# jianfch/stable-ts

Hardware: AMD Instinct MI355X
Metric: real-time factor (audio-sec/wall-sec) large-v3 word_timestamps=True (higher is better)
Workload: dtype f16; 1 GPU; large-v3 (random-init, weight recipe BENCH_WEIGHTS = the parity-pinned recipe of tests/test_gpu_f16_depth.py), 10 min synthetic 16 kHz audio per GPU, word_timestamps=True, beam_size=5, 112 decode steps/window, window-parallel batch 20, default regrouping inside the timed pass; mode=transcribe, windows_per_gpu=20, segments=125, words=1670, parallelism=dp1 (windows sharded, no data-path collective)

## Files before the change

### include/swx.h

```cpp
#ifndef SWX_H
#define SWX_H
#include <stdint.h>
#include <stddef.h>

#ifdef __cplusplus
extern "C" {
#endif

#define SWX_F32 0
#define SWX_F16 1

#define SWX_N_SAMPLES 480000
#define SWX_N_FRAMES 3000
#define SWX_N_FFT 400
#define SWX_HOP 160

typedef struct swx_dims {
    int32_t n_mels, n_audio_ctx, n_audio_state, n_audio_head, n_audio_layer;
    int32_t n_vocab, n_text_ctx, n_text_state, n_text_head, n_text_layer;
} swx_dims;

typedef struct swx_model swx_model;

const char *swx_strerror(int code);
// ... 131 lines not shown
int swx_flac_probe(const uint8_t *h_data, size_t n_bytes, swx_flac_info *info);
int64_t swx_flac_decode(const uint8_t *h_data, size_t n_bytes, int32_t *h_out, int64_t capacity_frames, swx_flac_info *info);

size_t swx_dtw_workspace_bytes(int W, int ld_n, int ld_m);
int swx_dtw(const float *d_x, int W, int ld_n, int ld_m, const int32_t *d_N, const int32_t *d_M,
            int32_t *d_text_idx, int32_t *d_time_idx, int32_t *d_len, void *d_trace_ws, void *stream);

int swx_prof_enable(int on);
int swx_debug_flags(int flags);
int swx_prof_collect(double *out, int n_classes);
int swx_graph_stats(const swx_model *m, int64_t *out);

int swx_test_gemm(int dtype, const void *d_a, int64_t lda, const void *d_w, const float *d_bias, const void *d_res,
                  void *d_c, int64_t ldc, int M, int N, int K, int epilogue, int force_kernel, void *stream);
int swx_test_gemm_plan(int M, int N, int K, int epilogue, int force_kernel, int flags);
int swx_test_dec_gemm(const void *d_a, int64_t lda, const void *d_w, const float *d_gamma, const float *d_beta,
                      const float *d_bias, void *d_c, int64_t ldc, void *d_x, void *d_kcache, void *d_vcache,
                      const int32_t *d_pos0, int n_ctx, int d, int M, int N, int K, int epilogue, void *d_scratch,
                      size_t scratch_bytes, void *stream);
int swx_test_layernorm(int dtype, const void *d_x, const float *d_g, const float *d_b, void *d_y, int rows, int d,
                       void *stream);
int swx_test_attention(int dtype, const void *d_q, int64_t ldq, const void *d_k, const void *d_v, int64_t ldkv,
                       void *d_o, int64_t ldo, int B, int H, int nq, int nk, int force_kernel, int vt_kp, void *stream);

int swx_test_gemm_layout(int dtype, const void *d_a, int64_t lda, const void *d_w, int64_t ldw, const float *d_bias, const void *d_res,
                         const float *d_resf, int res_mod, void *d_c, int64_t ldc, void *d_c2, void *d_p, int64_t p_bs, int p_nkpad,
                         int p_vcol0, int vt_s, int vt_kp, int64_t vt_bs, int vt_zero_pad, int M, int N, int K, int epilogue,
                         int force_kernel, void *stream);
int swx_test_xkv_pack(const void *d_k, const void *d_vt, void *d_packed, int B, int H, int nk, int ldk, int vt_kp, int64_t batch_stride,
                      void *stream);
// ... 56 lines not shown
```

### stable_ts_amd/_lib.py

```python
import ctypes
import os
from ctypes import POINTER, Structure, c_char_p, c_float, c_int, c_int32, c_int64, c_size_t, c_uint64, c_void_p

_HERE = os.path.dirname(os.path.abspath(__file__))
LIB_PATH = os.path.join(_HERE, "libswx.so")

SWX_F32 = 0
SWX_F16 = 1


class SwxError(RuntimeError):
    pass


class swx_dims(Structure):
    _fields_ = [(n, c_int32) for n in ("n_mels", "n_audio_ctx", "n_audio_state", "n_audio_head", "n_audio_layer",
                                       "n_vocab", "n_text_ctx", "n_text_state", "n_text_head", "n_text_layer")]


class swx_flac_info(Structure):
    _fields_ = [("sample_rate", c_int32), ("channels", c_int32), ("bits_per_sample", c_int32), ("min_block", c_int32),
                ("max_block", c_int32), ("total_samples", c_int64), ("md5", ctypes.c_uint8 * 16)]


# ... 79 lines not shown
    "swx_spectral_gate": (c_int, [c_void_p, c_int64, c_int, c_int64, POINTER(swx_gate_cfg), c_void_p, c_int64, c_void_p, c_size_t,
                                  c_void_p]),
    "swx_test_spectral_gate_block": (c_int, [c_int]),
    "swx_flac_probe": (c_int, [c_void_p, c_size_t, POINTER(swx_flac_info)]),
    "swx_flac_decode": (c_int64, [c_void_p, c_size_t, c_void_p, c_int64, POINTER(swx_flac_info)]),
    "swx_dtw_workspace_bytes": (c_size_t, [c_int, c_int, c_int]),
    "swx_dtw": (c_int, [c_void_p, c_int, c_int, c_int, c_void_p, c_void_p, c_void_p, c_void_p, c_void_p, c_void_p,
                        c_void_p]),
    "swx_prof_enable": (c_int, [c_int]),
    "swx_debug_flags": (c_int, [c_int]),
    "swx_prof_collect": (c_int, [POINTER(ctypes.c_double), c_int]),
    "swx_graph_stats": (c_int, [c_void_p, POINTER(c_int64)]),
    "swx_test_gemm": (c_int, [c_int, c_void_p, c_int64, c_void_p, c_void_p, c_void_p, c_void_p, c_int64, c_int, c_int,
                              c_int, c_int, c_int, c_void_p]),
    "swx_test_gemm_plan": (c_int, [c_int, c_int, c_int, c_int, c_int, c_int]),
    "swx_test_dec_gemm": (c_int, [c_void_p, c_int64, c_void_p, c_void_p, c_void_p, c_void_p, c_void_p, c_int64, c_void_p,
                                  c_void_p, c_void_p, c_void_p, c_int, c_int, c_int, c_int, c_int, c_int, c_void_p, c_size_t,
                                  c_void_p]),
    "swx_test_self_attn_step": (c_int, [c_void_p, c_void_p, c_void_p, c_void_p, c_void_p, c_int, c_int, c_int, c_int, c_int, c_void_p,
                                        c_void_p]),
    "swx_test_self_attn_multi": (c_int, [c_void_p, c_void_p, c_void_p, c_int, c_int, c_int, c_int, c_int, c_int, c_void_p, c_void_p]),
    "swx_test_self_attn_general": (c_int, [c_int, c_void_p, c_int64, c_void_p, c_void_p, c_void_p, c_void_p, c_int, c_int, c_int, c_int,
                                           c_int, c_int, c_int, c_int, c_void_p, c_void_p]),
    "swx_test_kcache_index": (c_int, [c_int] * 6),
    "swx_test_kcache_relayout": (c_int, [c_void_p, c_void_p, c_int64, c_int, c_int, c_int, c_int]),
    "swx_test_dec_gemm_kl": (c_int, [c_void_p, c_int64, c_void_p, c_void_p, c_void_p, c_void_p, c_void_p, c_int64, c_void_p,
                                     c_void_p, c_void_p, c_void_p, c_int, c_int, c_int, c_int, c_int, c_int, c_int, c_int, c_void_p,
                                     c_size_t, c_void_p]),
    "swx_test_self_attn_step_kl": (c_int, [c_void_p, c_void_p, c_void_p, c_void_p, c_void_p, c_int, c_int, c_int, c_int, c_int, c_int,
                                           c_void_p, c_void_p]),
# ... 64 lines not shown
```

### stable_ts_amd/csrc/swx_attn.hip

```cpp
#include <type_traits>
#include "swx_common.h"
#include "swx_kernels.h"
#include "swx_attn.h"

namespace {

constexpr int FL_KT = 64;
constexpr int FL_LD = 72;

template <bool VT, int QB>
__global__ __launch_bounds__(256, 2) void attn_flash2_f16(AttnArgs a)
{
    __shared__ __attribute__((aligned(16))) f16 Ks[2][FL_KT][FL_LD];
    __shared__ __attribute__((aligned(16))) f16 Vt[2][DH][FL_LD];
    const int tid = threadIdx.x, lane = tid & 63, wave = tid >> 6;
    const int b = blockIdx.z, h = blockIdx.y;
    const int q0 = blockIdx.x * (QB * 64) + wave * (QB * 16);
    const int qn = lane & 15, g = lane >> 4;
    const f16 *Q = (const f16 *)a.q;
    const f16 *K = (const f16 *)a.k + (size_t)b * a.k_bs + h * DH;
    const f16 *V = (const f16 *)a.v + (size_t)b * a.v_bs + (VT ? (size_t)h * DH * a.vt_kp : (size_t)h * DH);

    f16x8 qf[QB][2];
#pragma unroll
    for (int qb = 0; qb < QB; ++qb) {
// ... 68 lines not shown
            if (kt0 + FL_KT > a.nk) {
#pragma unroll
                for (int tt = 0; tt < 4; ++tt)
#pragma unroll
                    for (int r = 0; r < 4; ++r)
                        if (kt0 + tt * 16 + g * 4 + r >= a.nk) sc[tt][r] = -__builtin_inff();
            }
            float tmax = -__builtin_inff();
#pragma unroll
            for (int tt = 0; tt < 4; ++tt)
#pragma unroll
                for (int r = 0; r < 4; ++r) tmax = fmaxf(tmax, sc[tt][r]);
            tmax = lane_xor16_max(tmax);
            tmax = lane_xor32_max(tmax);
            const float m_new = fmaxf(m_run[qb], tmax);
            const float alpha = __builtin_amdgcn_exp2f((m_run[qb] - m_new) * SC2);
            const float mc = m_new * SC2;
            float psum = 0.f;
#pragma unroll
            for (int tt = 0; tt < 4; ++tt)
#pragma unroll
                for (int r = 0; r < 4; ++r) {
                    const float p = __builtin_amdgcn_exp2f(__builtin_fmaf(sc[tt][r], SC2, -mc));
                    sc[tt][r] = p;
                    psum += p;
                }
            psum = lane_xor16_add(psum);
            psum = lane_xor32_add(psum);
            l_run[qb] = l_run[qb] * alpha + psum;
            m_run[qb] = m_new;
#pragma unroll
            for (int tt = 0; tt < 4; ++tt) { o[qb][tt][0] *= alpha; o[qb][tt][1] *= alpha; o[qb][tt][2] *= alpha; o[qb][tt][3] *= alpha; }
#pragma unroll
            for (int c = 0; c < 2; ++c)
#pragma unroll
                for (int r = 0; r < 4; ++r) { pb[qb][c][r] = (f16)sc[2 * c][r]; pb[qb][c][4 + r] = (f16)sc[2 * c + 1][r]; }
        }
#pragma unroll
        for (int c = 0; c < 2; ++c)
#pragma unroll
            for (int tt = 0; tt < 4; ++tt) {
                const f16x4 lo = *(const f16x4 *)&Vt[cur][tt * 16 + qn][32 * c + g * 4];
                const f16x4 hi = *(const f16x4 *)&Vt[cur][tt * 16 + qn][32 * c + 16 + g * 4];
                f16x8 va;
#pragma unroll
                for (int e = 0; e < 4; ++e) { va[e] = lo[e]; va[4 + e] = hi[e]; }
#pragma unroll
// ... 503 lines not shown
                        part[(2 * RW_QB + qi) * DH + d] + part[(3 * RW_QB + qi) * DH + d];
        ((T *)a.o)[((size_t)b * a.q_rows_per_batch + q0 + qi) * a.ldo + h * DH + d] = from_f32<T>(v);
    }
}

}

static bool f32_flash_ready(bool vt, bool split)
{
    constexpr int need = (int)F32_LDS_BYTES;
    const hipError_t e = vt ? (split ? swx_lds_grant<attn_flash_f32<true, true>>(need) : swx_lds_grant<attn_flash_f32<true, false>>(need))
                            : (split ? swx_lds_grant<attn_flash_f32<false, true>>(need) : swx_lds_grant<attn_flash_f32<false, false>>(need));
    return e == hipSuccess;
}

int swx_attention(int dtype, const AttnArgs &a, int force_kernel, hipStream_t s)
{
    if (a.B <= 0 || a.nq <= 0 || a.nk <= 0) return 0;
    if (a.nk > RW_MAXK) return -5;
    const bool flash = (dtype == SWX_F16) && (force_kernel == 2 || (force_kernel >= 4 && force_kernel <= 6) || (force_kernel == 0 && a.nq >= 32));
    const size_t esz = dtype == SWX_F16 ? 2 : 4;
    const SwxXattnPlan xp = swx_xattn_plan(dtype, a, force_kernel, swx_flags());
    if (xp.family < 0) return xp.family;
    if (xp.family != SWX_XA_NOT_DECODE) return swx_xattn_launch(xp, a, s);
    if (flash) {
        if (dtype != SWX_F16) return -5;
        SwxProfScope prof(PC_ATTN_FLASH, 4.0 * a.B * a.H * (double)a.nq * a.nk * 64, s);
        const bool wide_fills = (int64_t)a.B * a.H * cdiv(a.nq, 256) >= 256;
        const bool narrow_fills = a.vt_kp && force_kernel == 0 && a.nq >= 256 && (int64_t)a.B * a.H * cdiv(a.nq, 128) <= 256 &&
                                  !(swx_flags() & SWX_FLAG_FLASH_NO_QB1);
        const int qb = !a.vt_kp ? 2 : narrow_fills ? 1 : force_kernel == 4 ? 2 : force_kernel == 6 ? 3 : (force_kernel == 5 || (a.nq >= 1024 && wide_fills)) ? 4 : 2;
        dim3 g(cdiv(a.nq, 64 * qb), a.H, a.B);
        const bool gen3 = a.vt_kp && (swx_flags() & SWX_FLAG_FLASH_PIPELINED);
        if (!a.vt_kp) hipLaunchKernelGGL((attn_flash2_f16<false, 2>), g, dim3(256), 0, s, a);
        else if (gen3 && qb == 4) hipLaunchKernelGGL((attn_flash3_f16<4>), g, dim3(256), 0, s, a);
        else if (gen3 && qb == 3) hipLaunchKernelGGL((attn_flash3_f16<3>), g, dim3(256), 0, s, a);
        else if (gen3 && qb == 2) hipLaunchKernelGGL((attn_flash3_f16<2>), g, dim3(256), 0, s, a);
        else if (qb == 4) hipLaunchKernelGGL((attn_flash2_f16<true, 4>), g, dim3(256), 0, s, a);
        else if (qb == 3) hipLaunchKernelGGL((attn_flash2_f16<true, 3>), g, dim3(256), 0, s, a);
        else if (qb == 1) hipLaunchKernelGGL((attn_flash2_f16<true, 1>), g, dim3(256), 0, s, a);
        else hipLaunchKernelGGL((attn_flash2_f16<true, 2>), g, dim3(256), 0, s, a);
    } else if (dtype == SWX_F32 && (force_kernel == 0 || force_kernel == 7) && a.vt_kp % F32_KT == 0 &&
               (a.vt_kp == 0 || a.vt_kp >= cdiv(a.nk, F32_KT) * F32_KT) && f32_flash_ready(a.vt_kp != 0, a.nq <= 16 && !a.f32_no_split)) {
        const bool split = a.nq <= 16 && !a.f32_no_split;
        SwxProfScope prof(split ? PC_ATTN_ROWWISE : PC_ATTN_FLASH,
                          split ? (double)a.B * a.H * 64 * esz * (2.0 * a.nk + 2.0 * a.nq) : 4.0 * a.B * a.H * (double)a.nq * a.nk * 64, s);
        dim3 gd(split ? 1 : cdiv(a.nq, 128), a.H, a.B);
        if (a.vt_kp) {
            if (split) hipLaunchKernelGGL((attn_flash_f32<true, true>), gd, dim3(256), F32_LDS_BYTES, s, a);
            else hipLaunchKernelGGL((attn_flash_f32<true, false>), gd, dim3(256), F32_LDS_BYTES, s, a);
        } else {
            if (split) hipLaunchKernelGGL((attn_flash_f32<false, true>), gd, dim3(256), F32_LDS_BYTES, s, a);
            else hipLaunchKernelGGL((attn_flash_f32<false, false>), gd, dim3(256), F32_LDS_BYTES, s, a);
        }
    } else {
        if (force_kernel == 7) return -5;
// ... 42 lines not shown
```

### stable_ts_amd/csrc/swx_gemm.hip

```cpp
#include "swx_gemm_tile.h"

namespace {

template <int MT>
__global__ __launch_bounds__(256) void gemm_f16_skinny(GemmArgs g)
{
    constexpr int NKS_MAX = 10;
    __shared__ f32x4 red[3][MT][64];
    const int tid = threadIdx.x, lane = tid & 63, wave = tid >> 6;
    const int n0 = blockIdx.x * 16;
    const f16 *A = (const f16 *)g.A;
    const f16 *W = (const f16 *)g.W;
    const int fr = lane & 15, fk = (lane >> 4) * 8;
    const int kslice = g.K / 4;
    const int nks = kslice / 32;
    const int kb = wave * kslice;
    const int n = n0 + fr;
    const bool nok = n < g.N;
    const f16 *wp = W + (size_t)(nok ? n : 0) * g.ldw + kb + fk;
    const f16x8 zero8 = (f16x8)(f16)0;

    f16x8 wf[NKS_MAX];
#pragma unroll
    for (int ks = 0; ks < NKS_MAX; ++ks) {
// ... 47 lines not shown
        }
    }
}

template <int MT = 1>
void launch_skinny(int mt, const GemmArgs &g, hipStream_t s)
{
    if constexpr (MT < 8) {
        if (mt > MT) return launch_skinny<MT + 1>(mt, g, s);
    }
    hipLaunchKernelGGL(gemm_f16_skinny<MT>, dim3(cdiv(g.N, 16)), dim3(256), 0, s, g);
}

}

int swx_gemm_plan_f16(int M, int N, int K, int epi, int64_t ldc, int64_t ldr, bool ptr16, int force_kernel, int flags)
{
    if (K % 32 != 0) return -4;
    const bool skinny_ok = M <= 128 && K % 128 == 0 && K / 128 <= 10 && N <= 16384;
    if (force_kernel == 2) return skinny_ok ? SWX_GEMM_SKINNY : -4;
    if (skinny_ok && force_kernel != 1 && force_kernel < 7) return SWX_GEMM_SKINNY;
    const bool glds_ok = K % 64 == 0 && ptr16;
    if (force_kernel >= 7 && !glds_ok) return -4;
    if (force_kernel == 1 || !glds_ok) return SWX_GEMM_TILED_REG;
    const int64_t t128 = (int64_t)cdiv(N, BN) * cdiv(M, BM);
    const bool narrow = force_kernel == 8 || (force_kernel != 9 && N % 64 == 0 && t128 < 224);
    const bool big_ok = !(epi & ~(EPI_BIAS | EPI_GELU | EPI_RES)) && ldc % 8 == 0 && (!(epi & EPI_RES) || ldr % 8 == 0);
    if (force_kernel == 12) return big_ok && K >= 128 ? SWX_GEMM_BIG : -4;
    const int64_t t256 = (int64_t)cdiv(M, BG) * cdiv(N, BG);
    const double fill = (double)t256 / (double)(((t256 + 255) / 256) * 256);
    if (force_kernel == 0 && big_ok && t256 >= 200 && K >= 512 && (fill >= 0.9 || (fill >= 0.75 && K >= 2560)) &&
        !(flags & SWX_FLAG_NO_BIG_TILE))
        return SWX_GEMM_BIG;
    const bool ring_ok = K >= 128;
    if (force_kernel == 10 || force_kernel == 11) return !ring_ok ? -4 : force_kernel == 10 ? SWX_GEMM_RING64 : SWX_GEMM_RING128;
    if (force_kernel == 0 && ring_ok && M > 256 && (narrow || t128 <= 256) && !(flags & SWX_FLAG_NO_RING))
        return narrow ? SWX_GEMM_RING64 : SWX_GEMM_RING128;
    return narrow ? SWX_GEMM_GLDS64 : SWX_GEMM_GLDS128;
}

int swx_gemm(int dtype, const GemmArgs &g, int force_kernel, hipStream_t s)
{
    if (g.M <= 0 || g.N <= 0) return 0;
    if (dtype == SWX_F16) {
        if (g.lda % 8 != 0 || g.ldw % 8 != 0) return -4;
        const bool ptr16 = (uintptr_t)g.A % 16 == 0 && (uintptr_t)g.W % 16 == 0;
        const bool cr16 = (uintptr_t)g.C % 16 == 0 && (!(g.epi & EPI_RES) || (uintptr_t)g.R % 16 == 0);
        const int plan = swx_gemm_plan_f16(g.M, g.N, g.K, g.epi, cr16 ? g.ldc : 1, cr16 ? g.ldr : 1, ptr16, force_kernel, swx_flags());
        if (plan < 0) return plan;
        if (plan == SWX_GEMM_SKINNY) {
            SwxProfScope prof(PC_GEMM_SKINNY, 2.0 * ((double)g.N * g.K + (double)g.M * g.K) + (double)g.M * g.N * ((g.epi & EPI_OUT_F32) ? 4 : 2), s);
            launch_skinny(cdiv(g.M, 16), g, s);
        } else {
            SwxProfScope prof(PC_GEMM_TILED, 2.0 * (double)g.M * g.N * g.K, s);
            if (const int rc = plan == SWX_GEMM_BIG ? swx_gemm_launch_big8(g, s) : swx_gemm_launch_tiled(plan, g, s)) return rc;
        }
    } else {
        if (g.K % 16 != 0 || g.lda % 4 != 0 || g.ldw % 4 != 0) return -4;
        SwxProfScope prof(PC_GEMM_TILED, 2.0 * (double)g.M * g.N * g.K, s);
        swx_gemm_launch_f32(g, force_kernel, s);
    }
    SWX_CHECK_LAUNCH();
    return 0;
}
```

### stable_ts_amd/csrc/swx_gemm_big.hip

```cpp
#include <type_traits>
#include "swx_gemm_tile.h"

namespace {

constexpr int BG_CLD = BG + 4;

__device__ __forceinline__ void big_tile_epilogue(const GemmArgs &g, unsigned char *ring, f32x4 (&acc)[8][4], int m0, int n0, int tid,
                                                  int lane, int wm, int wn)
{
    float (*Cs)[BG_CLD] = (float (*)[BG_CLD])ring;
    const int col_l = lane & 15, row_l = (lane >> 4) * 4;
    const int c8 = (tid & 31) * 8, rb = tid >> 5, gn = n0 + c8;
    const bool col_ok = gn < g.N, full = gn + 8 <= g.N;
    float bv[8];
#pragma unroll
    for (int e = 0; e < 8; ++e) bv[e] = ((g.epi & EPI_BIAS) && gn + e < g.N) ? g.bias[gn + e] : 0.f;
#pragma unroll
    for (int p = 0; p < 4; ++p) {
        f16x8 rv[4];
        if (g.epi & EPI_RES) {
#pragma unroll
            for (int it = 0; it < 4; ++it) {
                const int gm = m0 + p * 64 + it * 16 + rb;
                rv[it] = (gm < g.M && full) ? *(const f16x8 *)((const f16 *)g.R + (size_t)gm * g.ldr + gn) : (f16x8)(f16)0;
// ... 26 lines not shown
                    for (int e = 0; e < 8; ++e) v[e] += (float)rv[it][e];
                }
                f16x8 o;
#pragma unroll
                for (int e = 0; e < 8; ++e) o[e] = (f16)v[e];
                *(f16x8 *)cp = o;
            } else {
                for (int e = 0; e < 8 && gn + e < g.N; ++e) {
                    float t = v[e];
                    if (g.epi & EPI_RES) t += (float)((const f16 *)g.R)[(size_t)gm * g.ldr + gn + e];
                    cp[e] = (f16)t;
                }
            }
        }
        if (p < 3) __syncthreads();
    }
}

constexpr int B8_HALF = 128 * 128;
constexpr int B8_BUF = 4 * B8_HALF;

template <int N>
__device__ __forceinline__ void b8_wait_vm()
{
    asm volatile("s_waitcnt vmcnt(%0)" ::"n"(N) : "memory");
}
__device__ __forceinline__ void b8_barrier()
{
    asm volatile("s_barrier" ::: "memory");
}
// ... 126 lines not shown
        if (MODE == 0) issue(t + 2, I2());
        quad(I1(), I0(), fb0);
        b8_barrier();
    };

    issue(0, I0()); issue(0, I1()); issue(0, I2()); issue(0, I3());
    issue(1, I0()); issue(1, I1()); issue(1, I2());
    b8_wait_vm<10>();
    b8_barrier();
    if (wm_u == 1) b8_barrier();
    int t = 0;
    for (; t < KT - 2; ++t) tile(I0(), t);
    tile(I1(), t);
    tile(I2(), t + 1);
    if (wm_u == 0) b8_barrier();
    big_tile_epilogue(g, ring, acc, m0, n0, tid, lane, wm, wn);
}

}

int swx_gemm_launch_big8(const GemmArgs &g, hipStream_t s)
{
    GemmArgs gb = g;
    gb.tile_order = (swx_flags() & SWX_FLAG_BIG8_GROUPED) ? 1 : 0;
    return swx_launch_lds<gemm_f16_big8>(dim3(cdiv(g.N, BG), cdiv(g.M, BG)), dim3(512), 2 * B8_BUF, 2 * B8_BUF, s, gb);
}
```

### stable_ts_amd/csrc/swx_gemm_tile.h

```cpp
#pragma once
#include "swx_common.h"
#include "swx_kernels.h"

#define SWX_GEMM_LOCAL __attribute__((visibility("hidden")))
SWX_GEMM_LOCAL int swx_gemm_launch_tiled(int plan, const GemmArgs &g, hipStream_t s);
SWX_GEMM_LOCAL int swx_gemm_launch_big8(const GemmArgs &g, hipStream_t s);
SWX_GEMM_LOCAL void swx_gemm_launch_f32(const GemmArgs &g, int force_kernel, hipStream_t s);

constexpr int BM = 128, BN = 128;
constexpr int BK16 = 64, LD16 = BK16 + 8;
constexpr int GL_TILE = 128 * 128;
constexpr int BG = 256;

namespace {

template <typename T>
__device__ __forceinline__ void epilogue_store(const GemmArgs &g, int row, int col, float v)
{
    if (row >= g.M || col >= g.N) return;
    if (g.epi & EPI_BIAS) v += g.bias[col];
    if (g.epi & EPI_GELU) v = gelu_erf(v);
    if (g.epi & EPI_RESF32MOD) v += g.Rf[(size_t)(row % g.res_mod) * g.N + col];
    if (g.epi & EPI_RES) v += to_f32<T>(((const T *)g.R)[(size_t)row * g.ldr + col]);
    if (g.epi & EPI_STORE_VT) {
// ... 195 lines not shown
```

### stable_ts_amd/csrc/swx_kernels.h

```cpp
#pragma once
#include <hip/hip_runtime.h>
#include <stdint.h>
#include "../../include/swx.h"

#define EPI_BIAS 1
#define EPI_GELU 2
#define EPI_RES 4
#define EPI_OUT_F32 8
#define EPI_RESF32MOD 16
#define EPI_CBATCH 64
#define EPI_STORE_VT 32
#define EPI_KV 128

#define EPI_QKV_VT 256

struct GemmArgs {
    const void *A; int64_t lda;
    const void *W; int64_t ldw;
    const float *bias;
    const void *R; int64_t ldr;
    const float *Rf; int res_mod;
    void *C; int64_t ldc;
    void *C2;
    void *P; int64_t p_bs;
    int p_nkpad, p_vcol0;
    int M, N, K;
    int epi;
    int vt_s, vt_kp; int64_t vt_bs;
    int vt_zero_pad;
    int tile_order;
};
int swx_gemm(int dtype, const GemmArgs &g, int force_kernel, hipStream_t s);
enum { SWX_GEMM_TILED_REG = 0, SWX_GEMM_SKINNY = 1, SWX_GEMM_GLDS128 = 2, SWX_GEMM_GLDS64 = 3, SWX_GEMM_RING64 = 4, SWX_GEMM_RING128 = 5,
       SWX_GEMM_BIG = 6 };
int swx_gemm_plan_f16(int M, int N, int K, int epi, int64_t ldc, int64_t ldr, bool ptr16, int force_kernel, int flags);

#define SWX_FLAG_TABLE(X) \
    X(NO_FAST_STEP, 0)         \
    X(KCACHE_CHUNKED, 1)       \
    X(SELFATTN_NO_DEEP, 2)     \
    X(DEC_NO_W1, 4)            \
    X(TALL_NO_W8, 5)           \
    X(FLASH_NO_QB1, 6)         \
    X(XKV_PACK_SEPARATE, 7)    \
    X(SELFATTN_NO_MQ, 8)       \
    X(XQ_FULL_TILE, 9)         \
    X(DEC_W1_FULL_TILE, 10)    \
    X(NO_PACKED_XKV, 11)       \
    X(SELECT_MEM, 13)          \
    X(NO_GRAPH, 14)            \
    X(NO_PREFETCH, 15)         \
    X(NO_RING, 16)             \
    X(NO_BIG_TILE, 17)         \
    X(SCORE_TILED, 18)         \
    X(NO_TALL, 19)             \
    X(NO_FUSED_XQ, 20)         \
    X(TICKET, 21)              \
    X(BIG8_GROUPED, 22)        \
    X(XKV_TWO_LAUNCHES, 23)    \
    X(LOUDNESS_ONE_WG, 24)     \
    X(XATTN_R5, 25)            \
    X(FLASH_PIPELINED, 26)     \
    X(SELFATTN_WG5, 27)        \
    X(QKV_SEPARATE_VT, 28)
#define SWX_FLAG_DEFINE(name, bit) constexpr int SWX_FLAG_##name = 1 << (bit);
SWX_FLAG_TABLE(SWX_FLAG_DEFINE)
#undef SWX_FLAG_DEFINE
#define SWX_FLAG_IN_RANGE(name, bit) && (bit) >= 0 && (bit) <= 30
#define SWX_FLAG_OR(name, bit) | (int64_t(1) << (bit))
#define SWX_FLAG_SUM(name, bit) + (int64_t(1) << (bit))
static_assert(true SWX_FLAG_TABLE(SWX_FLAG_IN_RANGE), "SWX_FLAG_TABLE: a bit index outside 0..30");
static_assert((int64_t(0) SWX_FLAG_TABLE(SWX_FLAG_OR)) == (int64_t(0) SWX_FLAG_TABLE(SWX_FLAG_SUM)), "SWX_FLAG_TABLE: two switches share a bit");
#undef SWX_FLAG_IN_RANGE
#undef SWX_FLAG_OR
#undef SWX_FLAG_SUM
#define SWX_DEFAULT_FLAGS 0
int swx_flags();

struct KLayout { int sp, sh, sc; };
// ... 163 lines not shown
```

### stable_ts_amd/csrc/swx_runtime.hip

```cpp
#include <cmath>
#include <cstring>
#include <cstdio>
#include "swx_model.h"

namespace {

size_t add_slot(swx_model *m, size_t &cur, const std::string &name, int kind, int64_t rows, int64_t cols, int64_t dst_ld,
                size_t bytes, size_t base_off = (size_t)-1, size_t sub_off = 0)
{
    Slot s;
    s.kind = kind; s.rows = rows; s.cols = cols; s.dst_ld = dst_ld;
    if (base_off == (size_t)-1) { s.off = cur; cur = align_up(cur + bytes); }
    else s.off = base_off + sub_off;
    m->slots[name] = s;
    return s.off;
}

void build_layout(swx_model *m)
{
    const swx_dims &D = m->dims;
    const size_t e = m->esz;
    size_t cur = 0;
    auto mat = [&](const std::string &n, int64_t r, int64_t c) { return add_slot(m, cur, n, SK_MAT, r, c, c, (size_t)r * c * e); };
    auto vec = [&](const std::string &n, int64_t c) { return add_slot(m, cur, n, SK_VEC, 1, c, c, (size_t)c * 4); };
// ... 469 lines not shown
        unsigned char *c = h1 + ((size_t)b * 3002 + 1) * d * e;
        SWX_TRY(swx_gemm(m->dtype, swx_gemm_args(a, m->Cp, m->arena + m->o_conv1_w, 3 * m->Cp, m->A<float>(m->o_conv1_b), c, d,
                                             3000, d, 3 * m->Cp, EPI_BIAS | EPI_GELU), 0, s));
    }
    for (int b = 0; b < B; ++b) {
        const unsigned char *a = h1 + (size_t)b * 3002 * d * e;
        GemmArgs g = swx_gemm_args(a, 2 * d, m->arena + m->o_conv2_w, 3 * d, m->A<float>(m->o_conv2_b), x + (size_t)b * S_ * d * e, d,
                               S_, d, 3 * d, EPI_BIAS | EPI_GELU | EPI_RESF32MOD);
        g.Rf = m->A<float>(m->o_enc_pos); g.res_mod = S_;
        SWX_TRY(swx_gemm(m->dtype, g, 0, s));
    }
    for (int l = 0; l < D.n_audio_layer; ++l) {
        const LayerW &w = m->enc[l];
        SWX_TRY(swx_layernorm(m->dtype, x, d, m->A<float>(w.ln1_g), m->A<float>(w.ln1_b), h, d, rows, d, s));
        const bool fuse_vt = m->dtype == SWX_F16 && d % 128 == 0 && S_ % 4 == 0 && !(g_debug_flags & SWX_FLAG_QKV_SEPARATE_VT) &&
                             swx_gemm_plan_f16(rows, 3 * d, d, EPI_BIAS, 3 * d, 1, true, 0, g_debug_flags) != SWX_GEMM_BIG;
        {
            GemmArgs gq = swx_gemm_args(h, d, m->arena + w.wqkv, d, m->A<float>(w.bqkv), qkv, 3 * d, rows, 3 * d, d, EPI_BIAS | (fuse_vt ? EPI_QKV_VT : 0));
            if (fuse_vt) { gq.C2 = u; gq.vt_s = S_; gq.vt_kp = SWX_VT_KP; gq.vt_bs = (int64_t)H * 64 * SWX_VT_KP; gq.vt_zero_pad = 1; }
            SWX_TRY(swx_gemm(m->dtype, gq, 0, s));
        }
        AttnArgs a{};
        a.q = qkv; a.ldq = 3 * d; a.k = qkv + (size_t)d * e; a.v = qkv + (size_t)2 * d * e; a.ldkv = 3 * d; a.o = att; a.ldo = d;
        a.k_bs = (int64_t)S_ * 3 * d; a.v_bs = a.k_bs; a.vt_kp = 0;
        a.B = B; a.H = H; a.nq = S_; a.nk = S_; a.q_rows_per_batch = S_;
        if (m->dtype == SWX_F16) {
            if (!fuse_vt) SWX_TRY(swx_transpose_v(a.v, 3 * d, a.v_bs, S_, u, SWX_VT_KP, (int64_t)H * 64 * SWX_VT_KP, B, H, s));
            a.v = u; a.vt_kp = SWX_VT_KP; a.v_bs = (int64_t)H * 64 * SWX_VT_KP;
        }
        SWX_TRY(swx_attention(m->dtype, a, 0, s));
        SWX_TRY(swx_gemm_residual(m, att, d, w.wo, w.bo, x, d, rows, d, d, s));
// ... 69 lines not shown
```

### stable_ts_amd/csrc/swx_testhooks.hip

```cpp
#include <cstring>
#include "swx_model.h"

__global__ __launch_bounds__(64) void lane_xor_check_kernel(const uint32_t *__restrict__ in, uint32_t *__restrict__ out)
{
    const int lane = threadIdx.x;
    const uint32_t x = in[blockIdx.x * 64 + lane];
    uint32_t *o = out + (size_t)blockIdx.x * 13 * 64 + lane;
    o[0 * 64] = lane_xor_u32<32>(x, lane); o[1 * 64] = lane_xor_u32<16>(x, lane); o[2 * 64] = lane_xor_u32<8>(x, lane);
    o[3 * 64] = lane_xor_u32<4>(x, lane);  o[4 * 64] = lane_xor_u32<2>(x, lane);  o[5 * 64] = lane_xor_u32<1>(x, lane);
    o[6 * 64] = (uint32_t)__shfl_xor((int)x, 32, 64); o[7 * 64] = (uint32_t)__shfl_xor((int)x, 16, 64);
    o[8 * 64] = (uint32_t)__shfl_xor((int)x, 8, 64);  o[9 * 64] = (uint32_t)__shfl_xor((int)x, 4, 64);
    o[10 * 64] = (uint32_t)__shfl_xor((int)x, 2, 64); o[11 * 64] = (uint32_t)__shfl_xor((int)x, 1, 64);
    double v = (double)__uint_as_float(x);
    double ref = v;
#pragma unroll
    for (int off = 32; off > 0; off >>= 1) ref += __shfl_xor(ref, off, 64);
    const double got = wave_sum_d(v);
    unsigned ok = (__double_as_longlong(got) == __double_as_longlong(ref)) ? 1u : 0u;
    const float f = (float)(int)(x >> 9) * 1.1920929e-7f - 0.37f;
    ok |= (__float_as_uint(lane_xor16_max(f)) == __float_as_uint(fmaxf(f, __shfl_xor(f, 16, 64)))) ? 2u : 0u;
    ok |= (__float_as_uint(lane_xor32_max(f)) == __float_as_uint(fmaxf(f, __shfl_xor(f, 32, 64)))) ? 4u : 0u;
    ok |= (__float_as_uint(lane_xor16_add(f)) == __float_as_uint(f + __shfl_xor(f, 16, 64))) ? 8u : 0u;
    ok |= (__float_as_uint(lane_xor32_add(f)) == __float_as_uint(f + __shfl_xor(f, 32, 64))) ? 16u : 0u;
    float wm = f, ws = f;
// ... 56 lines not shown
    SWX_CHECK_LAUNCH();
    return 0;
}

int swx_test_gemm(int dtype, const void *d_a, int64_t lda, const void *d_w, const float *d_bias, const void *d_res,
                  void *d_c, int64_t ldc, int M, int N, int K, int epilogue, int force_kernel, void *stream)
{
    GemmArgs g = swx_gemm_args(d_a, lda, d_w, K, d_bias, d_c, ldc, M, N, K, epilogue);
    g.R = d_res; g.ldr = ldc;
    return swx_gemm(dtype, g, force_kernel, S(stream));
}

int swx_test_gemm_plan(int M, int N, int K, int epilogue, int force_kernel, int flags)
{
    return swx_gemm_plan_f16(M, N, K, epilogue, N, N, true, force_kernel, flags);
}

int swx_test_dec_gemm(const void *d_a, int64_t lda, const void *d_w, const float *d_gamma, const float *d_beta, const float *d_bias,
                      void *d_c, int64_t ldc, void *d_x, void *d_kcache, void *d_vcache, const int32_t *d_pos0, int n_ctx, int d,
                      int M, int N, int K, int epilogue, void *d_scratch, size_t scratch_bytes, void *stream)
{
    return swx_test_dec_gemm_kl(d_a, lda, d_w, d_gamma, d_beta, d_bias, d_c, ldc, d_x, d_kcache, d_vcache, d_pos0, n_ctx, d, M, N, K, epilogue,
                                0, 0, d_scratch, scratch_bytes, stream);
}

int swx_test_dec_gemm_kl(const void *d_a, int64_t lda, const void *d_w, const float *d_gamma, const float *d_beta, const float *d_bias,
                         void *d_c, int64_t ldc, void *d_x, void *d_kcache, void *d_vcache, const int32_t *d_pos0, int n_ctx, int d,
                         int M, int N, int K, int epilogue, int rps, int k_chunked, void *d_scratch, size_t scratch_bytes, void *stream)
{
    if (k_chunked && (epilogue & DEC_QKV) && (n_ctx <= 0 || d <= 0 || d % 64)) return -2;
// ... 167 lines not shown
{
    if (dtype != SWX_F16 && dtype != SWX_F32) return -1;
    if (!d_a || !d_w || !d_c || M <= 0 || N <= 0 || K <= 0 || lda <= 0 || ldw < K) return -1;
    if ((epilogue & EPI_BIAS) && !d_bias) return -1;
    if ((epilogue & EPI_RES) && !d_res) return -1;
    if ((epilogue & EPI_RESF32MOD) && (!d_resf || res_mod <= 0)) return -1;
    const int layout = epilogue & (EPI_CBATCH | EPI_STORE_VT | EPI_KV | EPI_QKV_VT);
    if (layout && vt_s <= 0) return -1;
    if ((epilogue & (EPI_STORE_VT | EPI_KV | EPI_QKV_VT)) && vt_kp < vt_s) return -1;
    if (layout & (layout - 1)) return -2;
    if (epilogue & (EPI_KV | EPI_QKV_VT)) {
        if (dtype != SWX_F16 || !d_c2) return -2;
        if ((epilogue & EPI_KV) ? N % 2 != 0 : N % 3 != 0) return -2;
        const int split = (epilogue & EPI_KV) ? N / 2 : (N / 3) * 2;
        const bool ptr16 = (uintptr_t)d_a % 16 == 0 && (uintptr_t)d_w % 16 == 0;
        const int plan = swx_gemm_plan_f16(M, N, K, epilogue, 1, 1, ptr16, force_kernel, swx_flags());
        if (plan < 0) return plan;
        if (plan == SWX_GEMM_SKINNY || plan == SWX_GEMM_BIG) return -2;
        const int width = (plan == SWX_GEMM_GLDS64 || plan == SWX_GEMM_RING64) ? 64 : 128;
        if (split % width != 0) return -2;
        if (vt_s % 4 != 0 || vt_kp % 4 != 0 || vt_bs % 4 != 0 || M % 4 != 0) return -2;
    } else if (vt_zero_pad) return -2;
    if (d_p) {
        if (!(epilogue & EPI_KV) || ldc % 8 != 0 || vt_bs % 8 != 0 || p_bs % 8 != 0 || p_vcol0 != N / 2) return -2;
        if (p_nkpad != ((vt_s + 31) / 32) * 32 || (epilogue & (EPI_RES | EPI_GELU | EPI_OUT_F32 | EPI_RESF32MOD))) return -2;
    }
    GemmArgs g = swx_gemm_args(d_a, lda, d_w, ldw, d_bias, d_c, ldc, M, N, K, epilogue);
    g.R = d_res; g.ldr = ldc; g.Rf = d_resf; g.res_mod = res_mod > 0 ? res_mod : 1;
    g.C2 = d_c2; g.P = d_p; g.p_bs = p_bs; g.p_nkpad = p_nkpad; g.p_vcol0 = p_vcol0;
    g.vt_s = vt_s; g.vt_kp = vt_kp; g.vt_bs = vt_bs; g.vt_zero_pad = vt_zero_pad ? 1 : 0;
    return swx_gemm(dtype, g, force_kernel, S(stream));
}

int swx_test_xkv_pack(const void *d_k, const void *d_vt, void *d_packed, int B, int H, int nk, int ldk, int vt_kp, int64_t batch_stride,
// ... 83 lines not shown
```

Measured before the change: 1442 x real time.

## Add f16 and fused V-transpose epilogues to big8 GEMM; trim flash softmax rescale

The big 256x256 GEMM gains an f16 epilogue that stages C through LDS as f16 and can write the V part of the QKV projection directly in transposed layout. The encoder can then use the big kernel together with the fused V-transpose instead of running a separate transpose or picking a smaller tile. The flash attention kernel also gets template variants that use packed FMA for the score scaling and skip the alpha rescale of o and l when the running max did not change for any lane of the wave. The cost is a larger LDS allocation for the big kernel, which may lower occupancy, and more template instantiations.

After: 1430 x real time. About the same (-0.8%).

```diff
diff --git a/include/swx.h b/include/swx.h
--- a/include/swx.h
+++ b/include/swx.h
@@ -169,6 +169,8 @@
 int swx_test_gemm(int dtype, const void *d_a, int64_t lda, const void *d_w, const float *d_bias, const void *d_res,
                   void *d_c, int64_t ldc, int M, int N, int K, int epilogue, int force_kernel, void *stream);
 int swx_test_gemm_plan(int M, int N, int K, int epilogue, int force_kernel, int flags);
+int swx_test_gemm_big8_epilogue(int N, int epilogue, int flags);
+int swx_test_transpose_v(const void *d_v, int64_t ldv, int64_t v_bs, int n, void *d_vt, int kp, int64_t vt_bs, int B, int H, void *stream);
 int swx_test_dec_gemm(const void *d_a, int64_t lda, const void *d_w, const float *d_gamma, const float *d_beta,
                       const float *d_bias, void *d_c, int64_t ldc, void *d_x, void *d_kcache, void *d_vcache,
                       const int32_t *d_pos0, int n_ctx, int d, int M, int N, int K, int epilogue, void *d_scratch,
diff --git a/stable_ts_amd/_lib.py b/stable_ts_amd/_lib.py
--- a/stable_ts_amd/_lib.py
+++ b/stable_ts_amd/_lib.py
@@ -117,6 +117,8 @@
     "swx_test_gemm": (c_int, [c_int, c_void_p, c_int64, c_void_p, c_void_p, c_void_p, c_void_p, c_int64, c_int, c_int,
                               c_int, c_int, c_int, c_void_p]),
     "swx_test_gemm_plan": (c_int, [c_int, c_int, c_int, c_int, c_int, c_int]),
+    "swx_test_gemm_big8_epilogue": (c_int, [c_int, c_int, c_int]),
+    "swx_test_transpose_v": (c_int, [c_void_p, c_int64, c_int64, c_int, c_void_p, c_int, c_int64, c_int, c_int, c_void_p]),
     "swx_test_dec_gemm": (c_int, [c_void_p, c_int64, c_void_p, c_void_p, c_void_p, c_void_p, c_void_p, c_int64, c_void_p,
                                   c_void_p, c_void_p, c_void_p, c_int, c_int, c_int, c_int, c_int, c_int, c_void_p, c_size_t,
                                   c_void_p]),
diff --git a/stable_ts_amd/csrc/swx_attn.hip b/stable_ts_amd/csrc/swx_attn.hip
--- a/stable_ts_amd/csrc/swx_attn.hip
+++ b/stable_ts_amd/csrc/swx_attn.hip
@@ -8,7 +8,7 @@
 constexpr int FL_KT = 64;
 constexpr int FL_LD = 72;
 
-template <bool VT, int QB>
+template <bool VT, int QB, int TRIM = 0>
 __global__ __launch_bounds__(256, 2) void attn_flash2_f16(AttnArgs a)
 {
     __shared__ __attribute__((aligned(16))) f16 Ks[2][FL_KT][FL_LD];
@@ -107,23 +107,37 @@
             tmax = lane_xor16_max(tmax);
             tmax = lane_xor32_max(tmax);
             const float m_new = fmaxf(m_run[qb], tmax);
-            const float alpha = __builtin_amdgcn_exp2f((m_run[qb] - m_new) * SC2);
             const float mc = m_new * SC2;
             float psum = 0.f;
 #pragma unroll
-            for (int tt = 0; tt < 4; ++tt)
+            for (int tt = 0; tt < 4; ++tt) {
+                if constexpr (TRIM & 1) {
+#pragma unroll
+                    for (int r = 0; r < 4; r += 2) {
+                        const f32x2 e = __builtin_elementwise_fma((f32x2){sc[tt][r], sc[tt][r + 1]}, (f32x2){SC2, SC2}, (f32x2){-mc, -mc});
+                        sc[tt][r] = e[0]; sc[tt][r + 1] = e[1];
+                    }
+                } else {
+#pragma unroll
+                    for (int r = 0; r < 4; ++r) sc[tt][r] = __builtin_fmaf(sc[tt][r], SC2, -mc);
+                }
 #pragma unroll
                 for (int r = 0; r < 4; ++r) {
-                    const float p = __builtin_amdgcn_exp2f(__builtin_fmaf(sc[tt][r], SC2, -mc));
+                    const float p = __builtin_amdgcn_exp2f(sc[tt][r]);
                     sc[tt][r] = p;
                     psum += p;
                 }
+            }
             psum = lane_xor16_add(psum);
             psum = lane_xor32_add(psum);
-            l_run[qb] = l_run[qb] * alpha + psum;
+            if (!(TRIM & 2) || __builtin_amdgcn_ballot_w64(m_new != m_run[qb]) != 0) {
+                const float alpha = __builtin_amdgcn_exp2f((m_run[qb] - m_new) * SC2);
+                l_run[qb] = l_run[qb] * alpha;
+#pragma unroll
+                for (int tt = 0; tt < 4; ++tt) { o[qb][tt][0] *= alpha; o[qb][tt][1] *= alpha; o[qb][tt][2] *= alpha; o[qb][tt][3] *= alpha; }
+            }
+            l_run[qb] = l_run[qb] + psum;
             m_run[qb] = m_new;
-#pragma unroll
-            for (int tt = 0; tt < 4; ++tt) { o[qb][tt][0] *= alpha; o[qb][tt][1] *= alpha; o[qb][tt][2] *= alpha; o[qb][tt][3] *= alpha; }
 #pragma unroll
             for (int c = 0; c < 2; ++c)
 #pragma unroll
@@ -657,11 +671,27 @@
     return e == hipSuccess;
 }
 
+template <int TRIM>
+static void flash2_vt_launch_qb(int qb, dim3 g, const AttnArgs &a, hipStream_t s)
+{
+    if (qb == 4) hipLaunchKernelGGL((attn_flash2_f16<true, 4, TRIM>), g, dim3(256), 0, s, a);
+    else if (qb == 3) hipLaunchKernelGGL((attn_flash2_f16<true, 3, TRIM>), g, dim3(256), 0, s, a);
+    else if (qb == 1) hipLaunchKernelGGL((attn_flash2_f16<true, 1, TRIM>), g, dim3(256), 0, s, a);
+    else hipLaunchKernelGGL((attn_flash2_f16<true, 2, TRIM>), g, dim3(256), 0, s, a);
+}
+static void flash2_vt_launch(int qb, int trim, dim3 g, const AttnArgs &a, hipStream_t s)
+{
+    if (trim == 3) flash2_vt_launch_qb<3>(qb, g, a, s);
+    else if (trim == 2) flash2_vt_launch_qb<2>(qb, g, a, s);
+    else if (trim == 1) flash2_vt_launch_qb<1>(qb, g, a, s);
+    else flash2_vt_launch_qb<0>(qb, g, a, s);
+}
+
 int swx_attention(int dtype, const AttnArgs &a, int force_kernel, hipStream_t s)
 {
     if (a.B <= 0 || a.nq <= 0 || a.nk <= 0) return 0;
     if (a.nk > RW_MAXK) return -5;
-    const bool flash = (dtype == SWX_F16) && (force_kernel == 2 || (force_kernel >= 4 && force_kernel <= 6) || (force_kernel == 0 && a.nq >= 32));
+    const bool flash = (dtype == SWX_F16) && (force_kernel == 2 || (force_kernel >= 4 && force_kernel <= 6) || force_kernel == 8 || (force_kernel == 0 && a.nq >= 32));
     const size_t esz = dtype == SWX_F16 ? 2 : 4;
     const SwxXattnPlan xp = swx_xattn_plan(dtype, a, force_kernel, swx_flags());
     if (xp.family < 0) return xp.family;
@@ -672,17 +702,14 @@
         const bool wide_fills = (int64_t)a.B * a.H * cdiv(a.nq, 256) >= 256;
         const bool narrow_fills = a.vt_kp && force_kernel == 0 && a.nq >= 256 && (int64_t)a.B * a.H * cdiv(a.nq, 128) <= 256 &&
                                   !(swx_flags() & SWX_FLAG_FLASH_NO_QB1);
-        const int qb = !a.vt_kp ? 2 : narrow_fills ? 1 : force_kernel == 4 ? 2 : force_kernel == 6 ? 3 : (force_kernel == 5 || (a.nq >= 1024 && wide_fills)) ? 4 : 2;
+        const int qb = !a.vt_kp ? 2 : (narrow_fills || force_kernel == 8) ? 1 : force_kernel == 4 ? 2 : force_kernel == 6 ? 3 : (force_kernel == 5 || (a.nq >= 1024 && wide_fills)) ? 4 : 2;
         dim3 g(cdiv(a.nq, 64 * qb), a.H, a.B);
         const bool gen3 = a.vt_kp && (swx_flags() & SWX_FLAG_FLASH_PIPELINED);
         if (!a.vt_kp) hipLaunchKernelGGL((attn_flash2_f16<false, 2>), g, dim3(256), 0, s, a);
         else if (gen3 && qb == 4) hipLaunchKernelGGL((attn_flash3_f16<4>), g, dim3(256), 0, s, a);
         else if (gen3 && qb == 3) hipLaunchKernelGGL((attn_flash3_f16<3>), g, dim3(256), 0, s, a);
         else if (gen3 && qb == 2) hipLaunchKernelGGL((attn_flash3_f16<2>), g, dim3(256), 0, s, a);
-        else if (qb == 4) hipLaunchKernelGGL((attn_flash2_f16<true, 4>), g, dim3(256), 0, s, a);
-        else if (qb == 3) hipLaunchKernelGGL((attn_flash2_f16<true, 3>), g, dim3(256), 0, s, a);
-        else if (qb == 1) hipLaunchKernelGGL((attn_flash2_f16<true, 1>), g, dim3(256), 0, s, a);
-        else hipLaunchKernelGGL((attn_flash2_f16<true, 2>), g, dim3(256), 0, s, a);
+        else flash2_vt_launch(qb, ((swx_flags() & SWX_FLAG_FLASH_NO_PK_FMA) ? 0 : 1) | ((swx_flags() & SWX_FLAG_FLASH_NO_SKIP) ? 0 : 2), g, a, s);
     } else if (dtype == SWX_F32 && (force_kernel == 0 || force_kernel == 7) && a.vt_kp % F32_KT == 0 &&
                (a.vt_kp == 0 || a.vt_kp >= cdiv(a.nk, F32_KT) * F32_KT) && f32_flash_ready(a.vt_kp != 0, a.nq <= 16 && !a.f32_no_split)) {
         const bool split = a.nq <= 16 && !a.f32_no_split;
diff --git a/stable_ts_amd/csrc/swx_gemm.hip b/stable_ts_amd/csrc/swx_gemm.hip
--- a/stable_ts_amd/csrc/swx_gemm.hip
+++ b/stable_ts_amd/csrc/swx_gemm.hip
@@ -85,6 +85,17 @@
 
 }
 
+int swx_gemm_big8_epilogue(int N, int epi, int flags)
+{
+    if (epi & EPI_QKV_VT) {
+        const bool ok = epi == (EPI_BIAS | EPI_QKV_VT) && N % 3 == 0 && ((N / 3) * 2) % BG == 0 &&
+                        !(flags & (SWX_FLAG_BIG8_NO_VT | SWX_FLAG_BIG8_F32_EPILOGUE));
+        return ok ? SWX_BIG8_EPI_F16_VT : -1;
+    }
+    if (epi & ~(EPI_BIAS | EPI_GELU | EPI_RES)) return -1;
+    return ((epi & EPI_BIAS) && !(epi & EPI_RES) && !(flags & SWX_FLAG_BIG8_F32_EPILOGUE)) ? SWX_BIG8_EPI_F16 : SWX_BIG8_EPI_F32;
+}
+
 int swx_gemm_plan_f16(int M, int N, int K, int epi, int64_t ldc, int64_t ldr, bool ptr16, int force_kernel, int flags)
 {
     if (K % 32 != 0) return -4;
@@ -96,7 +107,7 @@
     if (force_kernel == 1 || !glds_ok) return SWX_GEMM_TILED_REG;
     const int64_t t128 = (int64_t)cdiv(N, BN) * cdiv(M, BM);
     const bool narrow = force_kernel == 8 || (force_kernel != 9 && N % 64 == 0 && t128 < 224);
-    const bool big_ok = !(epi & ~(EPI_BIAS | EPI_GELU | EPI_RES)) && ldc % 8 == 0 && (!(epi & EPI_RES) || ldr % 8 == 0);
+    const bool big_ok = swx_gemm_big8_epilogue(N, epi, flags) >= 0 && ldc % 8 == 0 && (!(epi & EPI_RES) || ldr % 8 == 0);
     if (force_kernel == 12) return big_ok && K >= 128 ? SWX_GEMM_BIG : -4;
     const int64_t t256 = (int64_t)cdiv(M, BG) * cdiv(N, BG);
     const double fill = (double)t256 / (double)(((t256 + 255) / 256) * 256);
@@ -117,14 +128,17 @@
         if (g.lda % 8 != 0 || g.ldw % 8 != 0) return -4;
         const bool ptr16 = (uintptr_t)g.A % 16 == 0 && (uintptr_t)g.W % 16 == 0;
         const bool cr16 = (uintptr_t)g.C % 16 == 0 && (!(g.epi & EPI_RES) || (uintptr_t)g.R % 16 == 0);
-        const int plan = swx_gemm_plan_f16(g.M, g.N, g.K, g.epi, cr16 ? g.ldc : 1, cr16 ? g.ldr : 1, ptr16, force_kernel, swx_flags());
+        const bool vt4 = g.vt_s > 0 && g.vt_s % 4 == 0 && g.vt_kp % 4 == 0 && g.vt_bs % 4 == 0 && g.M % 4 == 0 && g.vt_kp >= g.vt_s &&
+                         g.C2 && (uintptr_t)g.C2 % 8 == 0;
+        const int flags = swx_flags() | (((g.epi & EPI_QKV_VT) && !vt4) ? SWX_FLAG_BIG8_NO_VT : 0);
+        const int plan = swx_gemm_plan_f16(g.M, g.N, g.K, g.epi, cr16 ? g.ldc : 1, cr16 ? g.ldr : 1, ptr16, force_kernel, flags);
         if (plan < 0) return plan;
         if (plan == SWX_GEMM_SKINNY) {
             SwxProfScope prof(PC_GEMM_SKINNY, 2.0 * ((double)g.N * g.K + (double)g.M * g.K) + (double)g.M * g.N * ((g.epi & EPI_OUT_F32) ? 4 : 2), s);
             launch_skinny(cdiv(g.M, 16), g, s);
         } else {
             SwxProfScope prof(PC_GEMM_TILED, 2.0 * (double)g.M * g.N * g.K, s);
-            if (const int rc = plan == SWX_GEMM_BIG ? swx_gemm_launch_big8(g, s) : swx_gemm_launch_tiled(plan, g, s)) return rc;
+            if (const int rc = plan == SWX_GEMM_BIG ? swx_gemm_launch_big8(g, flags, s) : swx_gemm_launch_tiled(plan, g, s)) return rc;
         }
     } else {
         if (g.K % 16 != 0 || g.lda % 4 != 0 || g.ldw % 4 != 0) return -4;
diff --git a/stable_ts_amd/csrc/swx_gemm_big.hip b/stable_ts_amd/csrc/swx_gemm_big.hip
--- a/stable_ts_amd/csrc/swx_gemm_big.hip
+++ b/stable_ts_amd/csrc/swx_gemm_big.hip
@@ -64,6 +64,69 @@
             }
         }
         if (p < 3) __syncthreads();
+    }
+}
+
+constexpr int BG_HLD = BG + 8;
+
+__device__ __forceinline__ void big_tile_epilogue_f16(const GemmArgs &g, unsigned char *ring, f32x4 (&acc)[8][4], int m0, int n0, int tid,
+                                                      int lane, int wave, int wm, int wn, bool vt)
+{
+    f16 (*Ch)[BG_HLD] = (f16 (*)[BG_HLD])ring;
+    const int col_l = lane & 15, row_l = (lane >> 4) * 4;
+    float bj[4];
+#pragma unroll
+    for (int j = 0; j < 4; ++j) {
+        const int gn = n0 + wn * 64 + j * 16 + col_l;
+        bj[j] = ((g.epi & EPI_BIAS) && gn < g.N) ? g.bias[gn] : 0.f;
+    }
+#pragma unroll
+    for (int i = 0; i < 8; ++i)
+#pragma unroll
+        for (int j = 0; j < 4; ++j) {
+            float v[4] = {acc[i][j][0] + bj[j], acc[i][j][1] + bj[j], acc[i][j][2] + bj[j], acc[i][j][3] + bj[j]};
+            if (g.epi & EPI_GELU) {
+                gelu_erf_n<4>(v);
+            }
+            const int row = wm * 128 + i * 16 + row_l, col = wn * 64 + j * 16 + col_l;
+            if (vt) {
+                const f16x4 o = {(f16)v[0], (f16)v[1], (f16)v[2], (f16)v[3]};
+                *(f16x4 *)&Ch[col][row] = o;
+            } else {
+#pragma unroll
+                for (int r = 0; r < 4; ++r) Ch[row + r][col] = (f16)v[r];
+            }
+        }
+    __syncthreads();
+    if (!vt) {
+        const int c8 = (tid & 31) * 8, rb = tid >> 5, gn = n0 + c8;
+        const bool col_ok = gn < g.N, full = gn + 8 <= g.N;
+#pragma unroll
+        for (int it = 0; it < 16; ++it) {
+            const int row = it * 16 + rb, gm = m0 + row;
+            if (gm >= g.M || !col_ok) continue;
+            const f16x8 o = *(const f16x8 *)&Ch[row][c8];
+            f16 *cp = (f16 *)g.C + (size_t)gm * g.ldc + gn;
+            if (full) *(f16x8 *)cp = o;
+            else for (int e = 0; e < 8 && gn + e < g.N; ++e) cp[e] = o[e];
+        }
+        return;
+    }
+    const int gm = m0 + lane * 4;
+    if (gm >= g.M) return;
+    const int split = (g.N / 3) * 2;
+    const int wb = gm / g.vt_s, sidx = gm - wb * g.vt_s;
+    f16 *cbase = (f16 *)g.C2 + (size_t)wb * g.vt_bs + sidx;
+    const bool pad = g.vt_zero_pad && sidx + 4 == g.vt_s;
+    for (int k = 0; k < 32; ++k) {
+        const int col = k * 8 + wave, gn = n0 + col;
+        if (gn >= g.N) break;
+        f16 *cp = cbase + (size_t)(gn - split) * g.vt_kp;
+        *(f16x4 *)cp = *(const f16x4 *)&Ch[col][lane * 4];
+        if (pad) {
+            const f16x4 z = {(f16)0.f, (f16)0.f, (f16)0.f, (f16)0.f};
+            for (int zp = 4; sidx + zp < g.vt_kp; zp += 4) *(f16x4 *)(cp + zp) = z;
+        }
     }
 }
 
@@ -220,14 +283,20 @@
     tile(I1(), t);
     tile(I2(), t + 1);
     if (wm_u == 0) b8_barrier();
-    big_tile_epilogue(g, ring, acc, m0, n0, tid, lane, wm, wn);
-}
-
-}
-
-int swx_gemm_launch_big8(const GemmArgs &g, hipStream_t s)
+    if (g.big_epi == SWX_BIG8_EPI_F32) big_tile_epilogue(g, ring, acc, m0, n0, tid, lane, wm, wn);
+    else big_tile_epilogue_f16(g, ring, acc, m0, n0, tid, lane, wave, wm, wn, g.big_epi == SWX_BIG8_EPI_F16_VT && n0 >= (g.N / 3) * 2);
+}
+
+}
+
+constexpr int B8_LDS = BG * BG_HLD * 2 > 2 * B8_BUF ? BG * BG_HLD * 2 : 2 * B8_BUF;
+static_assert(B8_LDS <= SWX_LDS_MAX, "the f16 epilogue tile has to fit a CU's LDS");
+
+int swx_gemm_launch_big8(const GemmArgs &g, int flags, hipStream_t s)
 {
     GemmArgs gb = g;
-    gb.tile_order = (swx_flags() & SWX_FLAG_BIG8_GROUPED) ? 1 : 0;
-    return swx_launch_lds<gemm_f16_big8>(dim3(cdiv(g.N, BG), cdiv(g.M, BG)), dim3(512), 2 * B8_BUF, 2 * B8_BUF, s, gb);
-}
+    gb.tile_order = (flags & SWX_FLAG_BIG8_GROUPED) ? 1 : 0;
+    gb.big_epi = swx_gemm_big8_epilogue(g.N, g.epi, flags);
+    if (gb.big_epi < 0) return -4;
+    return swx_launch_lds<gemm_f16_big8>(dim3(cdiv(g.N, BG), cdiv(g.M, BG)), dim3(512), B8_LDS, B8_LDS, s, gb);
+}
diff --git a/stable_ts_amd/csrc/swx_gemm_tile.h b/stable_ts_amd/csrc/swx_gemm_tile.h
--- a/stable_ts_amd/csrc/swx_gemm_tile.h
+++ b/stable_ts_amd/csrc/swx_gemm_tile.h
@@ -4,7 +4,7 @@
 
 #define SWX_GEMM_LOCAL __attribute__((visibility("hidden")))
 SWX_GEMM_LOCAL int swx_gemm_launch_tiled(int plan, const GemmArgs &g, hipStream_t s);
-SWX_GEMM_LOCAL int swx_gemm_launch_big8(const GemmArgs &g, hipStream_t s);
+SWX_GEMM_LOCAL int swx_gemm_launch_big8(const GemmArgs &g, int flags, hipStream_t s);
 SWX_GEMM_LOCAL void swx_gemm_launch_f32(const GemmArgs &g, int force_kernel, hipStream_t s);
 
 constexpr int BM = 128, BN = 128;
diff --git a/stable_ts_amd/csrc/swx_kernels.h b/stable_ts_amd/csrc/swx_kernels.h
--- a/stable_ts_amd/csrc/swx_kernels.h
+++ b/stable_ts_amd/csrc/swx_kernels.h
@@ -29,16 +29,20 @@
     int vt_s, vt_kp; int64_t vt_bs;
     int vt_zero_pad;
     int tile_order;
+    int big_epi;
 };
 int swx_gemm(int dtype, const GemmArgs &g, int force_kernel, hipStream_t s);
 enum { SWX_GEMM_TILED_REG = 0, SWX_GEMM_SKINNY = 1, SWX_GEMM_GLDS128 = 2, SWX_GEMM_GLDS64 = 3, SWX_GEMM_RING64 = 4, SWX_GEMM_RING128 = 5,
        SWX_GEMM_BIG = 6 };
 int swx_gemm_plan_f16(int M, int N, int K, int epi, int64_t ldc, int64_t ldr, bool ptr16, int force_kernel, int flags);
+enum { SWX_BIG8_EPI_F32 = 0, SWX_BIG8_EPI_F16 = 1, SWX_BIG8_EPI_F16_VT = 2 };
+int swx_gemm_big8_epilogue(int N, int epi, int flags);
 
 #define SWX_FLAG_TABLE(X) \
     X(NO_FAST_STEP, 0)         \
     X(KCACHE_CHUNKED, 1)       \
     X(SELFATTN_NO_DEEP, 2)     \
+    X(BIG8_F32_EPILOGUE, 3)    \
     X(DEC_NO_W1, 4)            \
     X(TALL_NO_W8, 5)           \
     X(FLASH_NO_QB1, 6)         \
@@ -47,6 +51,7 @@
     X(XQ_FULL_TILE, 9)         \
     X(DEC_W1_FULL_TILE, 10)    \
     X(NO_PACKED_XKV, 11)       \
+    X(BIG8_NO_VT, 12)          \
     X(SELECT_MEM, 13)          \
     X(NO_GRAPH, 14)            \
     X(NO_PREFETCH, 15)         \
@@ -62,7 +67,9 @@
     X(XATTN_R5, 25)            \
     X(FLASH_PIPELINED, 26)     \
     X(SELFATTN_WG5, 27)        \
-    X(QKV_SEPARATE_VT, 28)
+    X(QKV_SEPARATE_VT, 28)     \
+    X(FLASH_NO_PK_FMA, 29)     \
+    X(FLASH_NO_SKIP, 30)
 #define SWX_FLAG_DEFINE(name, bit) constexpr int SWX_FLAG_##name = 1 << (bit);
 SWX_FLAG_TABLE(SWX_FLAG_DEFINE)
 #undef SWX_FLAG_DEFINE
diff --git a/stable_ts_amd/csrc/swx_runtime.hip b/stable_ts_amd/csrc/swx_runtime.hip
--- a/stable_ts_amd/csrc/swx_runtime.hip
+++ b/stable_ts_amd/csrc/swx_runtime.hip
@@ -507,7 +507,8 @@
         const LayerW &w = m->enc[l];
         SWX_TRY(swx_layernorm(m->dtype, x, d, m->A<float>(w.ln1_g), m->A<float>(w.ln1_b), h, d, rows, d, s));
         const bool fuse_vt = m->dtype == SWX_F16 && d % 128 == 0 && S_ % 4 == 0 && !(g_debug_flags & SWX_FLAG_QKV_SEPARATE_VT) &&
-                             swx_gemm_plan_f16(rows, 3 * d, d, EPI_BIAS, 3 * d, 1, true, 0, g_debug_flags) != SWX_GEMM_BIG;
+                             (swx_gemm_plan_f16(rows, 3 * d, d, EPI_BIAS, 3 * d, 1, true, 0, g_debug_flags) != SWX_GEMM_BIG ||
+                              swx_gemm_plan_f16(rows, 3 * d, d, EPI_BIAS | EPI_QKV_VT, 3 * d, 1, true, 0, g_debug_flags) == SWX_GEMM_BIG);
         {
             GemmArgs gq = swx_gemm_args(h, d, m->arena + w.wqkv, d, m->A<float>(w.bqkv), qkv, 3 * d, rows, 3 * d, d, EPI_BIAS | (fuse_vt ? EPI_QKV_VT : 0));
             if (fuse_vt) { gq.C2 = u; gq.vt_s = S_; gq.vt_kp = SWX_VT_KP; gq.vt_bs = (int64_t)H * 64 * SWX_VT_KP; gq.vt_zero_pad = 1; }
diff --git a/stable_ts_amd/csrc/swx_testhooks.hip b/stable_ts_amd/csrc/swx_testhooks.hip
--- a/stable_ts_amd/csrc/swx_testhooks.hip
+++ b/stable_ts_amd/csrc/swx_testhooks.hip
@@ -94,6 +94,17 @@
 int swx_test_gemm_plan(int M, int N, int K, int epilogue, int force_kernel, int flags)
 {
     return swx_gemm_plan_f16(M, N, K, epilogue, N, N, true, force_kernel, flags);
+}
+
+int swx_test_gemm_big8_epilogue(int N, int epilogue, int flags)
+{
+    return swx_gemm_big8_epilogue(N, epilogue, flags);
+}
+
+int swx_test_transpose_v(const void *d_v, int64_t ldv, int64_t v_bs, int n, void *d_vt, int kp, int64_t vt_bs, int B, int H, void *stream)
+{
+    if (!d_v || !d_vt || ldv < 64 * (int64_t)H || ldv % 8 != 0 || v_bs % 8 != 0 || vt_bs % 8 != 0 || vt_bs < (int64_t)H * 64 * kp) return -1;
+    return swx_transpose_v(d_v, ldv, v_bs, n, d_vt, kp, vt_bs, B, H, S(stream));
 }
 
 int swx_test_dec_gemm(const void *d_a, int64_t lda, const void *d_w, const float *d_gamma, const float *d_beta, const float *d_bias,
@@ -291,10 +302,11 @@
         if ((epilogue & EPI_KV) ? N % 2 != 0 : N % 3 != 0) return -2;
         const int split = (epilogue & EPI_KV) ? N / 2 : (N / 3) * 2;
         const bool ptr16 = (uintptr_t)d_a % 16 == 0 && (uintptr_t)d_w % 16 == 0;
-        const int plan = swx_gemm_plan_f16(M, N, K, epilogue, 1, 1, ptr16, force_kernel, swx_flags());
+        const bool c16 = (uintptr_t)d_c % 16 == 0;
+        const int plan = swx_gemm_plan_f16(M, N, K, epilogue, c16 ? ldc : 1, 1, ptr16, force_kernel, swx_flags());
         if (plan < 0) return plan;
-        if (plan == SWX_GEMM_SKINNY || plan == SWX_GEMM_BIG) return -2;
-        const int width = (plan == SWX_GEMM_GLDS64 || plan == SWX_GEMM_RING64) ? 64 : 128;
+        if (plan == SWX_GEMM_SKINNY) return -2;
+        const int width = plan == SWX_GEMM_BIG ? 256 : (plan == SWX_GEMM_GLDS64 || plan == SWX_GEMM_RING64) ? 64 : 128;
         if (split % width != 0) return -2;
         if (vt_s % 4 != 0 || vt_kp % 4 != 0 || vt_bs % 4 != 0 || M % 4 != 0) return -2;
     } else if (vt_zero_pad) return -2;
```
